# W-Ted/F3D-Gaus

Measured on AMD Instinct MI355X. Metric: rendered views/sec at 256x256 (N Gaussians, K cams), higher is better.
Workload: dtype f32; 1 GPU; C2: 1 image/GPU, 196608 Gaussians (sigma0=0.01), 120-view orbit @256x256, GOF forward raster only; timed region = render + 8-bit RGB frames copied to pinned host memory; compositing arithmetic: fast = error-free float32 pairs for the float64 island + hardware exp/rcp/rsq; every channel within 1e-4 of the oracle (RGB <= 3e-7), EXCEPT that the distortion channel (values 1e-7..1e-5 from cancelling fl; gaussians=196608, views=120, resolution=256, tile_cull=1, views_per_call=120, render_mode=fast, channels=all, parallelism=single GPU

## Files before the change

### f3d-gaus_amd/csrc/f3dg_binning.hip

```cpp
#include "f3dg_common.h"

namespace {

typedef unsigned long long u64;
typedef unsigned int u32;

__global__ void __launch_bounds__(F3DG_BLOCK)
scan_reduce_kernel(const u32* __restrict__ in, u64 n, u32* __restrict__ block_sums)
{
    __shared__ u32 wsum[F3DG_BLOCK / 64];
    const u64 base = (u64)blockIdx.x * F3DG_SCAN_CHUNK;
    u32 s = 0;
#pragma unroll
    for (int i = 0; i < F3DG_SCAN_ITEMS; i++) {
        const u64 k = base + (u64)i * F3DG_BLOCK + threadIdx.x;
        if (k < n) s += in[k];
    }
#pragma unroll
    for (int off = 32; off > 0; off >>= 1) s += __shfl_down(s, off, 64);
    if ((threadIdx.x & 63) == 0) wsum[threadIdx.x >> 6] = s;
    __syncthreads();
    if (threadIdx.x == 0) block_sums[blockIdx.x] = wsum[0] + wsum[1] + wsum[2] + wsum[3];
}

__global__ void __launch_bounds__(1024)
scan_blocksums_kernel(u32* __restrict__ block_sums, u32 nblocks, F3dgHeader* __restrict__ hdr)
{
    __shared__ u32 wtot[16];
    __shared__ u32 carry_s;
    __shared__ u64 carry64_s, wtot64[16];
    if (threadIdx.x == 0) { carry_s = 0; carry64_s = 0; }
    __syncthreads();
    const int lane = threadIdx.x & 63, wave = threadIdx.x >> 6;
    for (u32 start = 0; start < nblocks; start += 1024) {
        const u32 i = start + threadIdx.x;
        const u32 v = i < nblocks ? block_sums[i] : 0;
        u32 x = v;
#pragma unroll
        for (int off = 1; off < 64; off <<= 1) {
            const u32 y = __shfl_up(x, off, 64);
            if (lane >= off) x += y;
        }
        if (lane == 63) wtot[wave] = x;
        unsigned long long v64 = v;
#pragma unroll
        for (int off = 32; off > 0; off >>= 1) v64 += __shfl_down(v64, off, 64);
        if (lane == 0) wtot64[wave] = v64;
        __syncthreads();
        u32 wave_off = 0;
        for (int w = 0; w < wave; w++) wave_off += wtot[w];
        const u32 carry = carry_s;
        if (i < nblocks) block_sums[i] = carry + wave_off + x - v;
        __syncthreads();
        if (threadIdx.x == 1023) {
            carry_s = carry + wave_off + x;
            u64 t = 0;
            for (int w = 0; w < 16; w++) t += wtot64[w];
            carry64_s += t;
        }
        __syncthreads();
    }
    if (hdr && threadIdx.x == 0) {
        const u64 total = carry64_s;
        hdr->num_rendered = total > 0xFFFFFFFFull ? 0xFFFFFFFFu : (u32)total;
        hdr->overflow = total > (u64)hdr->capacity ? 1u : 0u;
    }
}

__global__ void __launch_bounds__(F3DG_BLOCK)
scan_apply_kernel(const u32* in, u32* out , u64 n, const u32* __restrict__ block_sums,
                  int exclusive)
{
    __shared__ u32 wtot[F3DG_BLOCK / 64];
    const u64 base = (u64)blockIdx.x * F3DG_SCAN_CHUNK + (u64)threadIdx.x * F3DG_SCAN_ITEMS;
    u32 v[F3DG_SCAN_ITEMS];
    u32 s = 0;
    if (base + F3DG_SCAN_ITEMS <= n) {
#pragma unroll
        for (int i = 0; i < F3DG_SCAN_ITEMS / 4; i++) {
            const uint4 w = reinterpret_cast<const uint4*>(in + base)[i];
            v[4 * i] = w.x; v[4 * i + 1] = w.y; v[4 * i + 2] = w.z; v[4 * i + 3] = w.w;
        }
    } else {
#pragma unroll
        for (int i = 0; i < F3DG_SCAN_ITEMS; i++) v[i] = (base + i < n) ? in[base + i] : 0;
    }
#pragma unroll
    for (int i = 0; i < F3DG_SCAN_ITEMS; i++) s += v[i];
    const int lane = threadIdx.x & 63, wave = threadIdx.x >> 6;
    u32 x = s;
#pragma unroll
    for (int off = 1; off < 64; off <<= 1) {
        const u32 y = __shfl_up(x, off, 64);
        if (lane >= off) x += y;
    }
    if (lane == 63) wtot[wave] = x;
    __syncthreads();
    u32 run = block_sums[blockIdx.x] + x - s;
    for (int w = 0; w < wave; w++) run += wtot[w];
    u32 o[F3DG_SCAN_ITEMS];
#pragma unroll
    for (int i = 0; i < F3DG_SCAN_ITEMS; i++) {
        const u32 before = run;
        run += v[i];
        o[i] = exclusive ? before : run;
    }
    if (base + F3DG_SCAN_ITEMS <= n) {
#pragma unroll
        for (int i = 0; i < F3DG_SCAN_ITEMS / 4; i++)
            reinterpret_cast<uint4*>(out + base)[i] = make_uint4(o[4 * i], o[4 * i + 1], o[4 * i + 2], o[4 * i + 3]);
    } else {
#pragma unroll
        for (int i = 0; i < F3DG_SCAN_ITEMS; i++)
            if (base + i < n) out[base + i] = o[i];
    }
}


struct SegChunk {
    u64 seg_base;
    u64 obase;
    u32 n;
    u32 cps;
    u32 c;
    u32 seg;
};

struct SegTable {
    const u32* vstart;
    const u32* bglob;
    const u32* xprefix;
    u32 xstride;
    u32 V;
};

struct ShiftDigit {
    int shift;
    u32 mask = 255u;
    __device__ __forceinline__ u32 operator()(u32 k) const { return (k >> shift) & mask; }
};
struct CompactDigit {
    u32 kbase;
    __device__ __forceinline__ u32 operator()(u32 k) const { const u32 d = (k - kbase) >> 16; return d < 255u ? d : 255u; }
};

template <typename K, typename DIGIT, bool MINMAX = false>
__device__ __forceinline__ void hist_chunk(const K* __restrict__ keys, const SegChunk& ck, const DIGIT digit, u32* __restrict__ hist,
                                           u32 (*h)[256], u32* __restrict__ minmax = nullptr)
{
    u32 kmin = 0xFFFFFFFFu, kmax = 0u;
#pragma unroll
    for (int w = 0; w < F3DG_BLOCK / 64; w++) h[w][threadIdx.x] = 0;
    __syncthreads();
    u32* hw = h[threadIdx.x >> 6];
    constexpr int VEC = 16 / (int)sizeof(K);
    typedef K __attribute__((ext_vector_type(VEC))) KV;
    const u64 base = (u64)ck.c * F3DG_SORT_CHUNK;
    const u64 g0 = ck.seg_base + base;
    const u64 g1 = ck.seg_base + ((u64)ck.n - base < (u64)F3DG_SORT_CHUNK ? (u64)ck.n : base + F3DG_SORT_CHUNK);
    for (u64 a = (g0 & ~(u64)(VEC - 1)) + (u64)threadIdx.x * VEC; a < g1; a += (u64)F3DG_BLOCK * VEC) {
        const KV w = *reinterpret_cast<const KV*>(keys + a);
#pragma unroll
        for (int q = 0; q < VEC; q++) {
            if (a + q >= g0 && a + q < g1) {
                const u32 key = (u32)w[q];
                atomicAdd(&hw[digit(key)], 1u);
                if (MINMAX && key != 0xFFFFFFFFu) { kmin = key < kmin ? key : kmin; kmax = key > kmax ? key : kmax; }
            }
        }
    }
    __shared__ u32 wmm[2][F3DG_BLOCK / 64];
    if (MINMAX) {
#pragma unroll
        for (int off = 32; off > 0; off >>= 1) {
            const u32 a = __shfl_down(kmin, off, 64), b = __shfl_down(kmax, off, 64);
            kmin = a < kmin ? a : kmin; kmax = b > kmax ? b : kmax;
        }
        if ((threadIdx.x & 63) == 0) { wmm[0][threadIdx.x >> 6] = kmin; wmm[1][threadIdx.x >> 6] = kmax; }
    }
    __syncthreads();
    if (MINMAX && threadIdx.x == 0) {
        u32 a = wmm[0][0], b = wmm[1][0];
#pragma unroll
        for (int w = 1; w < F3DG_BLOCK / 64; w++) { a = wmm[0][w] < a ? wmm[0][w] : a; b = wmm[1][w] > b ? wmm[1][w] : b; }
        minmax[0] = a; minmax[1] = b;
    }
    hist[ck.obase + (u64)threadIdx.x * ck.cps + ck.c] = h[0][threadIdx.x] + h[1][threadIdx.x] + h[2][threadIdx.x] + h[3][threadIdx.x];
}

struct ScatterShared {
    u32 cnt[F3DG_BLOCK / 64][256];
    u32 lbase[256];
    u32 gdelta[256];
    u32 wtot[F3DG_BLOCK / 64];
    u32 sval[F3DG_SORT_CHUNK];
};

template <typename K, bool IOTA, typename DIGIT>
__device__ __forceinline__ void scatter_chunk(const K* __restrict__ keys_in, const u32* __restrict__ vals_in, K* __restrict__ keys_out,
                                              u32* __restrict__ vals_out, const SegChunk& ck, const DIGIT digit,
                                              const u32* __restrict__ offsets , ScatterShared& sh, K* skey)
{
    const u32 n = ck.n;
    const u64 block_base = (u64)ck.c * F3DG_SORT_CHUNK;
    const u32 in_block = (u32)((n - block_base) < (u64)F3DG_SORT_CHUNK ? (n - block_base) : (u64)F3DG_SORT_CHUNK);
    const int lane = threadIdx.x & 63, wave = threadIdx.x >> 6;
#pragma unroll
    for (int w = 0; w < F3DG_BLOCK / 64; w++) sh.cnt[w][threadIdx.x] = 0;
    __syncthreads();

    const u64 wave_base = block_base + (u64)wave * (64 * F3DG_SORT_ITEMS);
    u32 key[F3DG_SORT_ITEMS];
    u32 val[F3DG_SORT_ITEMS];
    u32 rank[F3DG_SORT_ITEMS];
    const u64 lane_lt = ((u64)1 << lane) - 1;
#pragma unroll
    for (int r = 0; r < F3DG_SORT_ITEMS; r++) {
        const u64 i = wave_base + (u64)r * 64 + lane;
        const bool valid = i < n;
        key[r] = valid ? (u32)keys_in[ck.seg_base + i] : 0u;
        val[r] = IOTA ? (u32)i : (valid ? vals_in[ck.seg_base + i] : 0u);
    }
#pragma unroll
    for (int r = 0; r < F3DG_SORT_ITEMS; r++) {
        const u64 i = wave_base + (u64)r * 64 + lane;
        const bool valid = i < n;
        const u32 d = digit(key[r]);
        u64 diff = 0;
#pragma unroll
        for (int b = 0; b < 8; b++) {
            const u32 own = (u32)((int)(d << (31 - b)) >> 31);
            const u64 bal = __ballot(own != 0u);
            diff |= bal ^ (((u64)own << 32) | own);
        }
        const u64 same = __ballot(valid) & ~diff;
        const u32 below = (u32)__popcll(same & lane_lt);
        const u32 prev = sh.cnt[wave][d];
        rank[r] = prev + below;
        __builtin_amdgcn_wave_barrier();
        if (valid && below == 0) sh.cnt[wave][d] = prev + (u32)__popcll(same);
        __builtin_amdgcn_wave_barrier();
    }
    __syncthreads();
    {
        const u32 d = threadIdx.x;
        const u32 c0 = sh.cnt[0][d], c1 = sh.cnt[1][d], c2 = sh.cnt[2][d], c3 = sh.cnt[3][d];
        const u32 tot = c0 + c1 + c2 + c3;
        u32 x = tot;
#pragma unroll
        for (int off = 1; off < 64; off <<= 1) {
            const u32 y = __shfl_up(x, off, 64);
            if (lane >= off) x += y;
        }
        if (lane == 63) sh.wtot[wave] = x;
        __syncthreads();
        u32 excl = x - tot;
        for (int w = 0; w < wave; w++) excl += sh.wtot[w];
        sh.lbase[d] = excl;
        sh.gdelta[d] = offsets[ck.obase + (u64)d * ck.cps + ck.c] - excl;
        sh.cnt[0][d] = excl;
        sh.cnt[1][d] = excl + c0;
        sh.cnt[2][d] = excl + c0 + c1;
        sh.cnt[3][d] = excl + c0 + c1 + c2;
    }
    __syncthreads();
#pragma unroll
    for (int r = 0; r < F3DG_SORT_ITEMS; r++) {
        const u64 i = wave_base + (u64)r * 64 + lane;
        if (i < n) {
            const u32 d = digit(key[r]);
            const u32 slot = sh.cnt[wave][d] + rank[r];
            skey[slot] = (K)key[r];
            sh.sval[slot] = val[r];
        }
    }
    __syncthreads();
    for (u32 slot = threadIdx.x; slot < in_block; slot += F3DG_BLOCK) {
        const K k = skey[slot];
        const u32 d = digit((u32)k);
        const u32 pos = sh.gdelta[d] + slot;
        if (keys_out) keys_out[pos] = k;
        vals_out[pos] = sh.sval[slot];
    }
}

__device__ __forceinline__ SegChunk fixed_chunk(u32 seg_len, u32 cps)
{
    u32 seg, c;
    f3dg_xcd_map(blockIdx.x, gridDim.x / cps, cps, seg, c);
    SegChunk ck;
    ck.seg_base = (u64)seg * seg_len; ck.obase = (u64)seg * 256u * cps; ck.n = seg_len; ck.cps = cps; ck.c = c; ck.seg = seg;
    return ck;
}

__device__ __forceinline__ bool gsort_compact(const u32* __restrict__ minmax, u32 view, u32& kbase)
{
    const u32 kmin = minmax[2 * view], kmax = minmax[2 * view + 1];
    kbase = kmin & 0xFFFF0000u;
    return kmin <= kmax && ((kmax - kbase) >> 24) == 0u;
}

template <int PASS>
__global__ void __launch_bounds__(F3DG_BLOCK)
gsort_hist_kernel(const u32* __restrict__ keys, u32 seg_len, u32 cps, u32* __restrict__ hist, const u32* __restrict__ minmax,
                  u32* __restrict__ chunk_minmax)
{
    __shared__ u32 h[F3DG_BLOCK / 64][256];
    const SegChunk ck = fixed_chunk(seg_len, cps);
    if constexpr (PASS == 0) {
        hist_chunk<u32, ShiftDigit>(keys, ck, ShiftDigit{0}, hist, h);
    } else if constexpr (PASS == 1) {
        hist_chunk<u32, ShiftDigit, true>(keys, ck, ShiftDigit{8}, hist, h, chunk_minmax + 2 * ((size_t)ck.seg * cps + ck.c));
    } else {
        u32 kbase;
        const bool compact = gsort_compact(minmax, ck.seg, kbase);
        if (!compact) {
            hist_chunk<u32, ShiftDigit>(keys, ck, ShiftDigit{8 * PASS}, hist, h);
        } else if constexpr (PASS == 2) {
            hist_chunk<u32, CompactDigit>(keys, ck, CompactDigit{kbase}, hist, h);
        } else {
            const u64 base = (u64)ck.c * F3DG_SORT_CHUNK;
            const u32 in_chunk = (u32)((ck.n - base) < (u64)F3DG_SORT_CHUNK ? (ck.n - base) : (u64)F3DG_SORT_CHUNK);
            hist[ck.obase + (u64)threadIdx.x * ck.cps + ck.c] = threadIdx.x == 0 ? in_chunk : 0u;
        }
    }
}

__global__ void __launch_bounds__(1024)
gsort_scan_kernel(u32 n_per_seg , u32 seg_len, u32* __restrict__ hist)
{
    __shared__ u32 wtot[16];
    __shared__ u32 carry_s;
    u32* h = hist + (size_t)blockIdx.x * n_per_seg;
    const u32 lane = threadIdx.x & 63u, wave = threadIdx.x >> 6;
    if (threadIdx.x == 0) carry_s = blockIdx.x * seg_len;
    __syncthreads();
    for (u32 base = 0; base < n_per_seg; base += 4096u) {
        const u32 i = base + 4u * threadIdx.x;
        uint4 v = make_uint4(0u, 0u, 0u, 0u);
        if (i < n_per_seg) v = *reinterpret_cast<const uint4*>(h + i);
        const u32 tot = v.x + v.y + v.z + v.w;
        u32 x = tot;
#pragma unroll
        for (int off = 1; off < 64; off <<= 1) {
            const u32 y = __shfl_up(x, off, 64);
            if (lane >= (u32)off) x += y;
        }
        if (lane == 63u) wtot[wave] = x;
        __syncthreads();
        u32 before = carry_s + x - tot;
        for (u32 w = 0; w < wave; w++) before += wtot[w];
        if (i < n_per_seg)
            *reinterpret_cast<uint4*>(h + i) = make_uint4(before, before + v.x, before + v.x + v.y, before + v.x + v.y + v.z);
        __syncthreads();
        if (threadIdx.x == 1023u) carry_s = before + tot;
        __syncthreads();
    }
}

__global__ void __launch_bounds__(64)
gsort_range_kernel(u32 cps, const u32* __restrict__ chunk_minmax, u32* __restrict__ minmax)
{
    u32 kmin = 0xFFFFFFFFu, kmax = 0u;
    for (u32 c = threadIdx.x; c < cps; c += 64) {
        const u32 a = chunk_minmax[2 * ((size_t)blockIdx.x * cps + c)], b = chunk_minmax[2 * ((size_t)blockIdx.x * cps + c) + 1];
        kmin = a < kmin ? a : kmin; kmax = b > kmax ? b : kmax;
    }
#pragma unroll
    for (int off = 32; off > 0; off >>= 1) {
        const u32 a = __shfl_down(kmin, off, 64), b = __shfl_down(kmax, off, 64);
        kmin = a < kmin ? a : kmin; kmax = b > kmax ? b : kmax;
    }
    if (threadIdx.x == 0) { minmax[2 * blockIdx.x] = kmin; minmax[2 * blockIdx.x + 1] = kmax; }
}

template <int PASS>
__global__ void __launch_bounds__(F3DG_BLOCK)
gsort_scatter_kernel(const u32* __restrict__ keys_in, const u32* __restrict__ vals_in, u32* __restrict__ keys_out,
                     u32* __restrict__ vals_out, u32 seg_len, u32 cps, const u32* __restrict__ offsets, const u32* __restrict__ minmax)
{
    __shared__ ScatterShared sh;
    __shared__ u32 skey[F3DG_SORT_CHUNK];
    const SegChunk ck = fixed_chunk(seg_len, cps);
    if constexpr (PASS == 0) {
        scatter_chunk<u32, true, ShiftDigit>(keys_in, vals_in, keys_out, vals_out, ck, ShiftDigit{0}, offsets, sh, skey);
    } else if constexpr (PASS == 1) {
        scatter_chunk<u32, false, ShiftDigit>(keys_in, vals_in, keys_out, vals_out, ck, ShiftDigit{8}, offsets, sh, skey);
    } else {
        u32 kbase;
        const bool compact = gsort_compact(minmax, ck.seg, kbase);
        if (!compact)
            scatter_chunk<u32, false, ShiftDigit>(keys_in, vals_in, PASS == 3 ? (u32*)nullptr : keys_out, vals_out, ck, ShiftDigit{8 * PASS}, offsets, sh, skey);
        else if constexpr (PASS == 2)
            scatter_chunk<u32, false, CompactDigit>(keys_in, vals_in, (u32*)nullptr, vals_out, ck, CompactDigit{kbase}, offsets, sh, skey);
    }
}

__global__ void __launch_bounds__(512)
view_segments_kernel(int V, int P, const u32* __restrict__ offsets_sorted, const F3dgHeader* __restrict__ hdr, u32* __restrict__ vstart,
                     u32* __restrict__ bglob, u32* __restrict__ xprefix, u32 xstride)
{
    __shared__ u32 carry;
    __shared__ u32 wtot[8];
    const u32 lane = threadIdx.x & 63u, wave = threadIdx.x >> 6;
    const bool dead = hdr->overflow != 0;
    auto start_of = [&](u32 v) -> u32 {
        const u64 i = (u64)v * (u64)P;
        return (dead || i == 0) ? 0u : offsets_sorted[i - 1];
    };
    auto chunks_of = [&](u32 v) -> u32 {
        const u32 n = start_of(v + 1) - start_of(v);
        return (n + F3DG_SORT_CHUNK - 1) / F3DG_SORT_CHUNK;
    };
    if (threadIdx.x == 0) carry = 0;
    __syncthreads();
    for (u32 v0 = 0; v0 < (u32)V; v0 += 512) {
        const u32 v = v0 + threadIdx.x;
        const u32 c = v < (u32)V ? chunks_of(v) : 0u;
        u32 x = c;
#pragma unroll
        for (int off = 1; off < 64; off <<= 1) {
            const u32 y = __shfl_up(x, off, 64);
            if (lane >= (u32)off) x += y;
        }
        if (lane == 63) wtot[wave] = x;
        __syncthreads();
        u32 woff = carry;
        for (u32 w = 0; w < wave; w++) woff += wtot[w];
        if (v < (u32)V) { vstart[v] = start_of(v); bglob[v] = woff + x - c; }
        __syncthreads();
        if (threadIdx.x == 511) carry = woff + x;
        __syncthreads();
    }
    if (threadIdx.x == 0) { vstart[V] = start_of((u32)V); bglob[V] = carry; }
    const u32 nk = ((u32)V > wave) ? ((u32)V - wave + 7u) / 8u : 0u;
    u32 run = 0;
    for (u32 k0 = 0; k0 < nk; k0 += 64) {
        const u32 k = k0 + lane;
        const u32 c = k < nk ? chunks_of(wave + 8u * k) : 0u;
        u32 x = c;
#pragma unroll
        for (int off = 1; off < 64; off <<= 1) {
            const u32 y = __shfl_up(x, off, 64);
            if (lane >= (u32)off) x += y;
        }
        if (k < nk) xprefix[wave * xstride + k] = run + x - c;
        run += __shfl(x, 63, 64);
    }
    if (lane == 0) xprefix[wave * xstride + nk] = run;
}

__global__ void __launch_bounds__(F3DG_BLOCK)
ranges_from_offsets_kernel(u32 V, u32 T, int tile_bits, const u32* __restrict__ bglob, const u32* __restrict__ offsets,
                           const F3dgHeader* __restrict__ hdr, uint2* __restrict__ ranges)
{
    const u32 i = blockIdx.x * F3DG_BLOCK + threadIdx.x;
    if (i >= V * T) return;
    const u32 v = i / T, t = i % T;
    const u32 b0 = bglob[v], cpv = bglob[v + 1] - b0;
    uint2 r = make_uint2(0u, 0u);
    if (cpv != 0u && !hdr->overflow) {
        const u32 d = ((v << tile_bits) | t) & 255u;
        const u32 lo = offsets[256ull * b0 + (u64)d * cpv], hi = offsets[256ull * b0 + (u64)(d + 1u) * cpv];
        if (hi > lo) r = make_uint2(lo, hi);
    }
    ranges[i] = r;
}

__device__ __forceinline__ bool var_chunk(const SegTable& st, u32 f, u32& k, SegChunk& ck)
{
    const u32 x = blockIdx.x & 7u;
    const u32* xp = st.xprefix + x * st.xstride;
    const u32 nk = (st.V > x) ? (st.V - x + 7u) / 8u : 0u;
    while (k < nk && f >= xp[k + 1]) k++;
    if (k >= nk) return false;
    const u32 v = x + 8u * k;
    const u32 s0 = st.vstart[v], b0 = st.bglob[v];
    ck.seg_base = s0; ck.n = st.vstart[v + 1] - s0; ck.cps = st.bglob[v + 1] - b0; ck.obase = 256ull * b0; ck.c = f - xp[k];
    return true;
}

template <typename K>
__global__ void __launch_bounds__(F3DG_BLOCK)
radix2_hist_var_kernel(const K* __restrict__ keys, SegTable st, int shift, u32 mask, u32* __restrict__ hist)
{
    __shared__ u32 h[F3DG_BLOCK / 64][256];
    u32 k = 0;
    SegChunk ck;
    for (u32 f = blockIdx.x >> 3; var_chunk(st, f, k, ck); f += gridDim.x >> 3)
        hist_chunk<K, ShiftDigit>(keys, ck, ShiftDigit{shift, mask}, hist, h);
}

template <typename K>
__global__ void __launch_bounds__(F3DG_BLOCK)
radix2_scatter_var_kernel(const K* __restrict__ keys_in, const u32* __restrict__ vals_in, K* __restrict__ keys_out,
                          u32* __restrict__ vals_out, SegTable st, int shift, u32 mask, const u32* __restrict__ offsets)
{
    __shared__ ScatterShared sh;
    __shared__ K skey[F3DG_SORT_CHUNK];
    u32 k = 0;
    SegChunk ck;
    for (u32 f = blockIdx.x >> 3; var_chunk(st, f, k, ck); f += gridDim.x >> 3) {
        scatter_chunk<K, false, ShiftDigit>(keys_in, vals_in, keys_out, vals_out, ck, ShiftDigit{shift, mask}, offsets, sh, skey);
        __syncthreads();
    }
}

__global__ void __launch_bounds__(F3DG_BLOCK)
gsort_gather_rects_kernel(int P, u32* __restrict__ gv0, u32* __restrict__ gv1, const u32* __restrict__ minmax,
                          const uint2* __restrict__ rects, u32* __restrict__ tiles_sorted, u32* __restrict__ rx)
{
    constexpr int ITEMS = 4;
    unsigned view, chunk;
    const unsigned cpv = (unsigned)((P + F3DG_BLOCK * ITEMS - 1) / (F3DG_BLOCK * ITEMS));
    f3dg_xcd_map(blockIdx.x, gridDim.x / cpv, cpv, view, chunk);
    const size_t vb = (size_t)view * P;
    u32 kbase;
    const bool pass2 = gsort_compact(minmax, view, kbase);
    const u32* perm = pass2 ? gv1 : gv0;
    u32* ry = pass2 ? gv0 : gv1;
    const int k0 = (int)(chunk * F3DG_BLOCK * ITEMS + threadIdx.x);
    u32 id[ITEMS];
    uint2 r[ITEMS];
#pragma unroll
    for (int i = 0; i < ITEMS; i++) { const int k = k0 + i * F3DG_BLOCK; id[i] = k < P ? perm[vb + k] : 0u; }
#pragma unroll
    for (int i = 0; i < ITEMS; i++) { const int k = k0 + i * F3DG_BLOCK; r[i] = k < P ? rects[vb + id[i]] : make_uint2(0u, 0u); }
#pragma unroll
    for (int i = 0; i < ITEMS; i++) {
        const int k = k0 + i * F3DG_BLOCK;
        if (k < P) {
            tiles_sorted[vb + k] = (((r[i].x >> 16) & F3DG_RECT_COORD) - (r[i].x & F3DG_RECT_COORD)) *
                                   (((r[i].y >> 16) & F3DG_RECT_COORD) - (r[i].y & F3DG_RECT_COORD));
            rx[vb + k] = r[i].x;
            ry[vb + k] = r[i].y;
        }
    }
}

#define F3DG_DUP_CAP 3072
template <typename G>
__global__ void __launch_bounds__(F3DG_BLOCK)
duplicate_sorted_kernel(int P, int tile_bits, int grid_x, const u32* __restrict__ gv0, const u32* __restrict__ gv1,
                        const u32* __restrict__ minmax, const u32* __restrict__ rx,
                        const u32* __restrict__ offsets_sorted,
                        const F3dgHeader* __restrict__ hdr, G* __restrict__ kgrp, u32* __restrict__ vals)
{
    __shared__ G sk[F3DG_DUP_CAP];
    __shared__ u32 sv[F3DG_DUP_CAP];
    if (hdr->overflow) return;
    const int k = blockIdx.x * F3DG_BLOCK + threadIdx.x;
    const int v = blockIdx.y;
    u32 kbase;
    const bool pass2 = gsort_compact(minmax, (u32)v, kbase);
    const u32* perm = pass2 ? gv1 : gv0;
    const u32* ry = pass2 ? gv0 : gv1;
    const size_t first = (size_t)v * P + (size_t)blockIdx.x * F3DG_BLOCK;
    const int in_block = min(F3DG_BLOCK, P - (int)(blockIdx.x * F3DG_BLOCK));
    const u32 base = first == 0 ? 0u : offsets_sorted[first - 1];
    const u32 n = offsets_sorted[first + in_block - 1] - base;
    u32 off0 = 0, cnt = 0, x = 0, y = 0, g = 0;
    if (k < P) {
        const size_t pos = (size_t)v * P + k;
        x = rx[pos]; y = ry[pos];
        const u32 rminx = x & F3DG_RECT_COORD, rmaxx = (x >> 16) & F3DG_RECT_COORD, rminy = y & F3DG_RECT_COORD, rmaxy = (y >> 16) & F3DG_RECT_COORD;
        if (rmaxx > rminx && rmaxy > rminy) {
            g = perm[pos];
            off0 = ((pos == 0) ? 0 : offsets_sorted[pos - 1]) - base;
            cnt = (rmaxx - rminx) * (rmaxy - rminy);
        }
    }
    const u32 rminx = x & F3DG_RECT_COORD, rmaxx = (x >> 16) & F3DG_RECT_COORD, rminy = y & F3DG_RECT_COORD, rmaxy = (y >> 16) & F3DG_RECT_COORD;
    const u32 view_base = (u32)v << tile_bits;
    auto halves = [](u32 t, u32 tmin, u32 tmax, u32 word) -> u32 {
        u32 m = 3u;
        if (t == tmin && (word & F3DG_RECT_SKIP_LO)) m &= ~1u;
        if (t + 1u == tmax && (word & F3DG_RECT_SKIP_HI)) m &= ~2u;
        return m;
    };
    for (u32 wb = 0; wb < n; wb += (u32)F3DG_DUP_CAP) {
        const u32 lo = off0 > wb ? off0 : wb;
        const u32 hi = off0 + cnt < wb + (u32)F3DG_DUP_CAP ? off0 + cnt : wb + (u32)F3DG_DUP_CAP;
        if (lo < hi) {
            const u32 w = rmaxx - rminx, j0 = lo - off0;
            u32 ty = rminy + j0 / w, tx = rminx + j0 % w;
            u32 my = halves(ty, rminy, rmaxy, y);
            for (u32 j = lo; j < hi; j++) {
                const u32 mx = halves(tx, rminx, rmaxx, x);
                sk[j - wb] = (G)(view_base | (ty * (u32)grid_x + tx));
                sv[j - wb] = g | ((((my & 1u) ? mx : 0u) | ((my & 2u) ? mx << 2 : 0u)) << F3DG_ID_BITS);
                if (++tx == rmaxx) { tx = rminx; ty++; my = halves(ty, rminy, rmaxy, y); }
            }
        }
        __syncthreads();
        const u32 in_win = n - wb < (u32)F3DG_DUP_CAP ? n - wb : (u32)F3DG_DUP_CAP;
        for (u32 i = threadIdx.x; i < in_win; i += F3DG_BLOCK) {
            kgrp[base + wb + i] = sk[i];
            vals[base + wb + i] = sv[i];
        }
        __syncthreads();
    }
}

__global__ void __launch_bounds__(F3DG_BLOCK)
export_keys_kernel(u32 nseg, int P, int tile_bits, int T, const uint2* __restrict__ ranges, const F3dgHeader* __restrict__ hdr,
                   const u32* __restrict__ point_list, const float* __restrict__ depths, u64* __restrict__ keys_out)
{
    if (hdr->overflow) return;
    for (u32 seg = blockIdx.x; seg < nseg; seg += gridDim.x) {
        const uint2 r = ranges[seg];
        const u32 view = seg / (u32)T, tile = seg % (u32)T;
        const u64 hi = (u64)((view << tile_bits) | tile) << 32;
        for (u32 i = r.x + threadIdx.x; i < r.y; i += F3DG_BLOCK)
            keys_out[i] = hi | (u64)__float_as_uint(depths[(size_t)view * P + (point_list[i] & F3DG_ID_MASK)]);
    }
}

template <typename G>
__global__ void __launch_bounds__(F3DG_BLOCK)
group_bounds_kernel(const G* __restrict__ kgrp, const F3dgHeader* __restrict__ hdr, int tile_bits, int T, u32* __restrict__ ranges)
{
    const u32 L = hdr->overflow ? 0u : hdr->num_rendered;
    const u32 tmask = (1u << tile_bits) - 1u;
    for (u64 base = ((u64)blockIdx.x * F3DG_BLOCK + threadIdx.x) * 8u; base < L; base += (u64)gridDim.x * F3DG_BLOCK * 8u) {
        G v[8];
        if (base + 8 <= L) {
            typedef G __attribute__((ext_vector_type(8))) G8;
            const G8 w = *reinterpret_cast<const G8*>(kgrp + base);
#pragma unroll
            for (int i = 0; i < 8; i++) v[i] = w[i];
        } else {
#pragma unroll
            for (int i = 0; i < 8; i++) v[i] = base + i < L ? kgrp[base + i] : (G)0;
        }
        u32 prev = base > 0 ? (u32)kgrp[base - 1] : 0u;
        const u32 next = base + 8 < L ? (u32)kgrp[base + 8] : 0u;
#pragma unroll
        for (int i = 0; i < 8; i++) {
            const u64 idx = base + i;
            if (idx < L) {
                const u32 cur = (u32)v[i];
                const u32 nxt = i < 7 ? (u32)v[i + 1] : next;
                const u32 seg = (cur >> tile_bits) * (u32)T + (cur & tmask);
                if (idx == 0 || prev != cur) ranges[2u * seg] = (u32)idx;
                if (idx == L - 1 || nxt != cur) ranges[2u * seg + 1u] = (u32)idx + 1u;
                prev = cur;
            }
        }
    }
}

int bits_for(unsigned long long n_values)
{
    int b = 0;
    while (b < 64 && (n_values - 1) >> b) b++;
    return n_values <= 1 ? 0 : b;
}

}

int f3dg_launch_scan_inclusive(hipStream_t s, const unsigned* in, unsigned* out, unsigned long long n,
                               unsigned* tmp, unsigned tmp_elems, int exclusive, F3dgHeader* hdr_total)
{
    if (n == 0) return F3DG_OK;
    const unsigned nblocks = (unsigned)((n + F3DG_SCAN_CHUNK - 1) / F3DG_SCAN_CHUNK);
    if (nblocks > tmp_elems) return F3DG_ERR_WORKSPACE;
    F3DG_KLAUNCH(scan_reduce_kernel, dim3(nblocks), dim3(F3DG_BLOCK), 0, s, in, (u64)n, tmp);
    F3DG_KLAUNCH(scan_blocksums_kernel, dim3(1), dim3(1024), 0, s, tmp, nblocks, hdr_total);
    F3DG_KLAUNCH(scan_apply_kernel, dim3(nblocks), dim3(F3DG_BLOCK), 0, s, in, out, (u64)n, tmp, exclusive);
    F3DG_HIP_CHECK(hipGetLastError());
    return F3DG_OK;
}

int f3dg_tile_bits(int T) { return bits_for((unsigned long long)T); }


int f3dg_sort_passes(int V, int T)
{
    (void)V;
    const int bits = f3dg_tile_bits(T);
    return bits == 0 ? 0 : (bits + 7) / 8;
}

template <typename G>
static int binning_tail(hipStream_t s, int V, int P, int grid_x, int T, int tile_bits, const F3dgLayout& L, char* ws, F3dgHeader* hdr)
{
    int rc = F3DG_OK;
    const size_t VP = (size_t)V * P;
    u32* scan_tmp = reinterpret_cast<u32*>(ws + L.scan_tmp);
    u32* hist = reinterpret_cast<u32*>(ws + L.hist);
    u32* gk[2] = { reinterpret_cast<u32*>(ws + L.gsort), reinterpret_cast<u32*>(ws + L.gsort) + VP };
    u32* gv[2] = { reinterpret_cast<u32*>(ws + L.gsort) + 2 * VP, reinterpret_cast<u32*>(ws + L.gsort) + 3 * VP };
    G* kgrp[2] = { reinterpret_cast<G*>(ws + L.keys[0]), reinterpret_cast<G*>(ws + L.keys[1]) };
    u32* vals[2] = { reinterpret_cast<u32*>(ws + L.vals[0]), reinterpret_cast<u32*>(ws + L.vals[1]) };
    const dim3 pgrid((P + F3DG_BLOCK - 1) / F3DG_BLOCK, V);

    const u32 cps = (u32)((P + F3DG_SORT_CHUNK - 1) / F3DG_SORT_CHUNK);
    const u32 gblocks = (u32)V * cps;
    u32* minmax = reinterpret_cast<u32*>(ws + L.segtab) + L.segtab_minmax;
    u32* chunk_minmax = minmax + 2 * (size_t)V;
    const bool view_scan = cps <= 64;
#define F3DG_GSORT_PASS(PASS, IN, OUT)                                                                                                     \
    F3DG_KLAUNCH((gsort_hist_kernel<PASS>), dim3(gblocks), dim3(F3DG_BLOCK), 0, s, gk[IN], (u32)P, cps, hist, minmax, chunk_minmax); \
    if (view_scan)                                                                                                                         \
        F3DG_KLAUNCH(gsort_scan_kernel, dim3(V), dim3(1024), 0, s, 256u * cps, (u32)P, hist);                                       \
    else {                                                                                                                                 \
        rc = f3dg_launch_scan_inclusive(s, hist, hist, (unsigned long long)256 * gblocks, scan_tmp, L.scan_tmp_elems, 1, nullptr);        \
        if (rc != F3DG_OK) return rc;                                                                                                      \
    }                                                                                                                                      \
    F3DG_KLAUNCH((gsort_scatter_kernel<PASS>), dim3(gblocks), dim3(F3DG_BLOCK), 0, s, gk[IN], gv[IN], gk[OUT], gv[OUT], (u32)P, cps, hist, minmax)
    F3DG_GSORT_PASS(0, 0, 1);
    F3DG_GSORT_PASS(1, 1, 0);
    F3DG_KLAUNCH(gsort_range_kernel, dim3(V), dim3(64), 0, s, cps, chunk_minmax, minmax);
    F3DG_GSORT_PASS(2, 0, 1);
    F3DG_GSORT_PASS(3, 1, 0);
#undef F3DG_GSORT_PASS
    u32* offsets_sorted = gk[1];
    u32* rx = gk[0];

    F3DG_KLAUNCH(gsort_gather_rects_kernel, dim3((unsigned)V * (unsigned)((P + 4 * F3DG_BLOCK - 1) / (4 * F3DG_BLOCK))), dim3(F3DG_BLOCK), 0, s, P, gv[0], gv[1], minmax,
                           reinterpret_cast<const uint2*>(ws + L.rects), offsets_sorted, rx);
    rc = f3dg_launch_scan_inclusive(s, offsets_sorted, offsets_sorted, (unsigned long long)VP, scan_tmp, L.scan_tmp_elems, 0, hdr);
    if (rc != F3DG_OK) return rc;
    const int passes = f3dg_sort_passes(V, T);
    int src = passes & 1;
    F3DG_KLAUNCH((duplicate_sorted_kernel<G>), pgrid, dim3(F3DG_BLOCK), 0, s, P, tile_bits, grid_x, gv[0], gv[1], minmax, rx, offsets_sorted, hdr,
                       kgrp[src], vals[src]);

    if (passes > 0) {
        SegTable st;
        u32* segtab = reinterpret_cast<u32*>(ws + L.segtab);
        const u32 xstride = (u32)V / 8u + 2u;
        st.vstart = segtab; st.bglob = segtab + (V + 1); st.xprefix = segtab + 2 * (V + 1); st.xstride = xstride; st.V = (u32)V;
        F3DG_KLAUNCH(view_segments_kernel, dim3(1), dim3(512), 0, s, V, P, offsets_sorted, hdr, segtab, segtab + (V + 1),
                           segtab + 2 * (V + 1), xstride);
        const size_t nbmax = (size_t)L.sort_blocks + (size_t)V;
        const u32 per_xcd = (u32)((nbmax + 7) / 8 < 160 ? (nbmax + 7) / 8 : 160);
        const u32 per_xcd_h = (u32)((nbmax + 7) / 8 < 512 ? (nbmax + 7) / 8 : 512);
        const int split = passes == 2 ? (tile_bits + 1) / 2 : 8;
        for (int p = 0; p < passes; p++) {
            const int shift = split * p;
            const u32 mask = passes == 2 ? (1u << (p == 0 ? split : tile_bits - split)) - 1u : 255u;
            F3DG_HIP_CHECK(hipMemsetAsync(hist, 0, sizeof(u32) * 256 * nbmax, s));
            F3DG_KLAUNCH((radix2_hist_var_kernel<G>), dim3(8 * per_xcd_h), dim3(F3DG_BLOCK), 0, s, kgrp[src], st, shift, mask, hist);
            rc = f3dg_launch_scan_inclusive(s, hist, hist, (unsigned long long)256 * nbmax, scan_tmp, L.scan_tmp_elems, 1, nullptr);
            if (rc != F3DG_OK) return rc;
            F3DG_KLAUNCH((radix2_scatter_var_kernel<G>), dim3(8 * per_xcd), dim3(F3DG_BLOCK), 0, s, kgrp[src], vals[src],
                               passes == 1 ? (G*)nullptr : kgrp[src ^ 1], vals[src ^ 1], st, shift, mask, hist);
            src ^= 1;
        }
        if (passes == 1) {
            const u32 nseg = (u32)V * (u32)T;
            F3DG_KLAUNCH(ranges_from_offsets_kernel, dim3((nseg + F3DG_BLOCK - 1) / F3DG_BLOCK), dim3(F3DG_BLOCK), 0, s, (u32)V, (u32)T, tile_bits,
                               segtab + (V + 1), hist, hdr, reinterpret_cast<uint2*>(ws + L.ranges));
            F3DG_HIP_CHECK(hipGetLastError());
            return F3DG_OK;
        }
    }
    F3DG_HIP_CHECK(hipMemsetAsync(ws + L.ranges, 0, sizeof(uint2) * (size_t)V * T, s));
    F3DG_KLAUNCH((group_bounds_kernel<G>), dim3(2048), dim3(F3DG_BLOCK), 0, s, kgrp[0], hdr, tile_bits, T, reinterpret_cast<u32*>(ws + L.ranges));
    F3DG_HIP_CHECK(hipGetLastError());
    return F3DG_OK;
}

int f3dg_launch_binning(hipStream_t s, int V, int P, int W, int H, const F3dgLayout& L, char* ws, int export_offsets)
{
    const int grid_x = (W + F3DG_TILE - 1) / F3DG_TILE, grid_y = (H + F3DG_TILE - 1) / F3DG_TILE;
    const int T = grid_x * grid_y;
    const int tile_bits = f3dg_tile_bits(T);
    F3dgHeader* hdr = reinterpret_cast<F3dgHeader*>(ws + L.header);

    int rc = F3DG_OK;
    if (export_offsets) {
        rc = f3dg_launch_scan_inclusive(s, reinterpret_cast<const u32*>(ws + L.tiles), reinterpret_cast<u32*>(ws + L.offsets),
                                        (unsigned long long)V * P, reinterpret_cast<u32*>(ws + L.scan_tmp), L.scan_tmp_elems, 0, nullptr);
        if (rc != F3DG_OK) return rc;
    }
    const bool small = (((unsigned long long)(V > 0 ? V - 1 : 0) << tile_bits) | ((1ull << tile_bits) - 1ull)) <= 0xFFFFull;
    rc = small ? binning_tail<unsigned short>(s, V, P, grid_x, T, tile_bits, L, ws, hdr)
               : binning_tail<u32>(s, V, P, grid_x, T, tile_bits, L, ws, hdr);
    if (rc != F3DG_OK) return rc;
    F3DG_HIP_CHECK(hipGetLastError());
    return F3DG_OK;
}

int f3dg_launch_export_keys(hipStream_t s, int V, int P, int W, int H, const F3dgLayout& L, char* ws)
{
    const int grid_x = (W + F3DG_TILE - 1) / F3DG_TILE, grid_y = (H + F3DG_TILE - 1) / F3DG_TILE;
    const int T = grid_x * grid_y;
    const u32 nseg = (u32)V * (u32)T;
    const u32 rg = nseg < 65535u * 4u ? nseg : 65535u * 4u;
    F3DG_KLAUNCH(export_keys_kernel, dim3(rg), dim3(F3DG_BLOCK), 0, s, nseg, P, f3dg_tile_bits(T), T,
                       reinterpret_cast<const uint2*>(ws + L.ranges), reinterpret_cast<const F3dgHeader*>(ws + L.header),
                       reinterpret_cast<const u32*>(ws + L.vals[0]), reinterpret_cast<const float*>(ws + L.depths),
                       reinterpret_cast<u64*>(ws + L.keys[0]));
    F3DG_HIP_CHECK(hipGetLastError());
    return F3DG_OK;
}
```

Baseline: 29990 views/s.

## Replace global per-Gaussian offset scan with block sums and per-view segmented scans

Drops the full V*P inclusive scan of per-Gaussian tile counts. The gather kernel now writes per-block sums, a per-view kernel scans those, view totals feed view_segments, and the duplicate kernel rebuilds intra-block offsets with a wave scan. It also swaps the global scan of the tile radix histograms for a per-view tile_scan kernel, which skips the memset, and skips the redundant pass-3 scan for compact views. The aim is fewer launches and less global memory traffic in binning, at the cost of more complex bookkeeping, overflow detection moved into view_segments, and memset elision that relies on the histogram kernel fully writing its range.

```diff
diff --git a/f3d-gaus_amd/csrc/f3dg_binning.hip b/f3d-gaus_amd/csrc/f3dg_binning.hip
--- a/f3d-gaus_amd/csrc/f3dg_binning.hip
+++ b/f3d-gaus_amd/csrc/f3dg_binning.hip
@@ -303,7 +303,7 @@
 template <int PASS>
 __global__ void __launch_bounds__(F3DG_BLOCK)
 gsort_hist_kernel(const u32* __restrict__ keys, u32 seg_len, u32 cps, u32* __restrict__ hist, const u32* __restrict__ minmax,
-                  u32* __restrict__ chunk_minmax)
+                  u32* __restrict__ chunk_minmax, int standin )
 {
     __shared__ u32 h[F3DG_BLOCK / 64][256];
     const SegChunk ck = fixed_chunk(seg_len, cps);
@@ -318,7 +318,7 @@
             hist_chunk<u32, ShiftDigit>(keys, ck, ShiftDigit{8 * PASS}, hist, h);
         } else if constexpr (PASS == 2) {
             hist_chunk<u32, CompactDigit>(keys, ck, CompactDigit{kbase}, hist, h);
-        } else {
+        } else if (standin) {
             const u64 base = (u64)ck.c * F3DG_SORT_CHUNK;
             const u32 in_chunk = (u32)((ck.n - base) < (u64)F3DG_SORT_CHUNK ? (ck.n - base) : (u64)F3DG_SORT_CHUNK);
             hist[ck.obase + (u64)threadIdx.x * ck.cps + ck.c] = threadIdx.x == 0 ? in_chunk : 0u;
@@ -327,10 +327,12 @@
 }
 
 __global__ void __launch_bounds__(1024)
-gsort_scan_kernel(u32 n_per_seg , u32 seg_len, u32* __restrict__ hist)
+gsort_scan_kernel(u32 n_per_seg , u32 seg_len, u32* __restrict__ hist, const u32* __restrict__ skip_compact )
 {
     __shared__ u32 wtot[16];
     __shared__ u32 carry_s;
+    u32 kbase;
+    if (skip_compact && gsort_compact(skip_compact, blockIdx.x, kbase)) return;
     u32* h = hist + (size_t)blockIdx.x * n_per_seg;
     const u32 lane = threadIdx.x & 63u, wave = threadIdx.x >> 6;
     if (threadIdx.x == 0) carry_s = blockIdx.x * seg_len;
@@ -396,20 +398,87 @@
     }
 }
 
+
+__global__ void __launch_bounds__(1024)
+block_sums_scan_kernel(u32 nb, u32* __restrict__ block_sums, u64* __restrict__ view_total)
+{
+    __shared__ u32 wtot[16];
+    __shared__ u32 carry_s;
+    __shared__ u64 carry64_s, wtot64[16];
+    u32* b = block_sums + (size_t)blockIdx.x * nb;
+    const u32 lane = threadIdx.x & 63u, wave = threadIdx.x >> 6;
+    if (threadIdx.x == 0) { carry_s = 0; carry64_s = 0; }
+    __syncthreads();
+    for (u32 start = 0; start < nb; start += 1024u) {
+        const u32 i = start + threadIdx.x;
+        const u32 v = i < nb ? b[i] : 0u;
+        u32 x = v;
+#pragma unroll
+        for (int off = 1; off < 64; off <<= 1) {
+            const u32 y = __shfl_up(x, off, 64);
+            if (lane >= (u32)off) x += y;
+        }
+        if (lane == 63u) wtot[wave] = x;
+        u64 v64 = v;
+#pragma unroll
+        for (int off = 32; off > 0; off >>= 1) v64 += __shfl_down(v64, off, 64);
+        if (lane == 0u) wtot64[wave] = v64;
+        __syncthreads();
+        u32 before = carry_s + x - v;
+        for (u32 w = 0; w < wave; w++) before += wtot[w];
+        if (i < nb) b[i] = before;
+        __syncthreads();
+        if (threadIdx.x == 1023u) {
+            carry_s = before + v;
+            u64 t = 0;
+            for (int w = 0; w < 16; w++) t += wtot64[w];
+            carry64_s += t;
+        }
+        __syncthreads();
+    }
+    if (threadIdx.x == 0) view_total[blockIdx.x] = carry64_s;
+}
+
 __global__ void __launch_bounds__(512)
-view_segments_kernel(int V, int P, const u32* __restrict__ offsets_sorted, const F3dgHeader* __restrict__ hdr, u32* __restrict__ vstart,
+view_segments_kernel(int V, const u64* __restrict__ view_total, F3dgHeader* __restrict__ hdr, u32* __restrict__ vstart,
                      u32* __restrict__ bglob, u32* __restrict__ xprefix, u32 xstride)
 {
     __shared__ u32 carry;
     __shared__ u32 wtot[8];
+    __shared__ u64 carry64, wtot64[8];
     const u32 lane = threadIdx.x & 63u, wave = threadIdx.x >> 6;
-    const bool dead = hdr->overflow != 0;
-    auto start_of = [&](u32 v) -> u32 {
-        const u64 i = (u64)v * (u64)P;
-        return (dead || i == 0) ? 0u : offsets_sorted[i - 1];
-    };
+    if (threadIdx.x == 0) carry64 = 0;
+    __syncthreads();
+    for (u32 v0 = 0; v0 < (u32)V; v0 += 512) {
+        const u32 v = v0 + threadIdx.x;
+        const u64 t = v < (u32)V ? view_total[v] : 0ull;
+        u64 x = t;
+#pragma unroll
+        for (int off = 1; off < 64; off <<= 1) {
+            const u64 y = __shfl_up(x, off, 64);
+            if (lane >= (u32)off) x += y;
+        }
+        if (lane == 63) wtot64[wave] = x;
+        __syncthreads();
+        u64 woff = carry64;
+        for (u32 w = 0; w < wave; w++) woff += wtot64[w];
+        if (v < (u32)V) vstart[v] = (u32)(woff + x - t);
+        __syncthreads();
+        if (threadIdx.x == 511) carry64 = woff + x;
+        __syncthreads();
+    }
+    const u64 total = carry64;
+    const bool dead = total > (u64)hdr->capacity;
+    if (threadIdx.x == 0) {
+        hdr->num_rendered = total > 0xFFFFFFFFull ? 0xFFFFFFFFu : (u32)total;
+        hdr->overflow = dead ? 1u : 0u;
+        vstart[V] = dead ? 0u : (u32)total;
+    }
+    if (dead)
+        for (u32 v = threadIdx.x; v < (u32)V; v += 512) vstart[v] = 0u;
+    __syncthreads();
     auto chunks_of = [&](u32 v) -> u32 {
-        const u32 n = start_of(v + 1) - start_of(v);
+        const u32 n = vstart[v + 1] - vstart[v];
         return (n + F3DG_SORT_CHUNK - 1) / F3DG_SORT_CHUNK;
     };
     if (threadIdx.x == 0) carry = 0;
@@ -427,12 +496,12 @@
         __syncthreads();
         u32 woff = carry;
         for (u32 w = 0; w < wave; w++) woff += wtot[w];
-        if (v < (u32)V) { vstart[v] = start_of(v); bglob[v] = woff + x - c; }
+        if (v < (u32)V) bglob[v] = woff + x - c;
         __syncthreads();
         if (threadIdx.x == 511) carry = woff + x;
         __syncthreads();
     }
-    if (threadIdx.x == 0) { vstart[V] = start_of((u32)V); bglob[V] = carry; }
+    if (threadIdx.x == 0) bglob[V] = carry;
     const u32 nk = ((u32)V > wave) ? ((u32)V - wave + 7u) / 8u : 0u;
     u32 run = 0;
     for (u32 k0 = 0; k0 < nk; k0 += 64) {
@@ -448,6 +517,53 @@
         run += __shfl(x, 63, 64);
     }
     if (lane == 0) xprefix[wave * xstride + nk] = run;
+}
+
+__global__ void __launch_bounds__(1024)
+tile_scan_kernel(u32 V, const u32* __restrict__ vstart, const u32* __restrict__ bglob, u32* __restrict__ hist)
+{
+    constexpr u32 ITEMS = 16;
+    __shared__ u32 wtot[16];
+    __shared__ u32 carry_s;
+    const u32 b0 = bglob[blockIdx.x], n = 256u * (bglob[blockIdx.x + 1] - b0);
+    u32* h = hist + 256ull * b0;
+    const u32 lane = threadIdx.x & 63u, wave = threadIdx.x >> 6;
+    if (blockIdx.x == 0 && threadIdx.x == 0) hist[256ull * bglob[V]] = vstart[V];
+    if (threadIdx.x == 0) carry_s = vstart[blockIdx.x];
+    __syncthreads();
+    for (u32 base = 0; base < n; base += 1024u * ITEMS) {
+        const u32 i = base + ITEMS * threadIdx.x;
+        u32 v[ITEMS];
+#pragma unroll
+        for (u32 q = 0; q < ITEMS / 4; q++) {
+            const uint4 w = i < n ? reinterpret_cast<const uint4*>(h + i)[q] : make_uint4(0u, 0u, 0u, 0u);
+            v[4 * q] = w.x; v[4 * q + 1] = w.y; v[4 * q + 2] = w.z; v[4 * q + 3] = w.w;
+        }
+        u32 tot = 0;
+#pragma unroll
+        for (u32 q = 0; q < ITEMS; q++) tot += v[q];
+        u32 x = tot;
+#pragma unroll
+        for (int off = 1; off < 64; off <<= 1) {
+            const u32 y = __shfl_up(x, off, 64);
+            if (lane >= (u32)off) x += y;
+        }
+        if (lane == 63u) wtot[wave] = x;
+        __syncthreads();
+        u32 run = carry_s + x - tot;
+        for (u32 w = 0; w < wave; w++) run += wtot[w];
+        if (i < n) {
+#pragma unroll
+            for (u32 q = 0; q < ITEMS / 4; q++) {
+                uint4 o;
+                o.x = run; run += v[4 * q]; o.y = run; run += v[4 * q + 1]; o.z = run; run += v[4 * q + 2]; o.w = run; run += v[4 * q + 3];
+                reinterpret_cast<uint4*>(h + i)[q] = o;
+            }
+        }
+        __syncthreads();
+        if (threadIdx.x == 1023u) carry_s = run;
+        __syncthreads();
+    }
 }
 
 __global__ void __launch_bounds__(F3DG_BLOCK)
@@ -506,11 +622,18 @@
     }
 }
 
+__device__ __forceinline__ u32 rect_instances(u32 x, u32 y)
+{
+    const u32 rminx = x & F3DG_RECT_COORD, rmaxx = (x >> 16) & F3DG_RECT_COORD, rminy = y & F3DG_RECT_COORD, rmaxy = (y >> 16) & F3DG_RECT_COORD;
+    return (rmaxx > rminx && rmaxy > rminy) ? (rmaxx - rminx) * (rmaxy - rminy) : 0u;
+}
+
 __global__ void __launch_bounds__(F3DG_BLOCK)
 gsort_gather_rects_kernel(int P, u32* __restrict__ gv0, u32* __restrict__ gv1, const u32* __restrict__ minmax,
-                          const uint2* __restrict__ rects, u32* __restrict__ tiles_sorted, u32* __restrict__ rx)
+                          const uint2* __restrict__ rects, u32* __restrict__ block_sums, u32* __restrict__ rx)
 {
     constexpr int ITEMS = 4;
+    __shared__ u32 wsum[ITEMS][F3DG_BLOCK / 64];
     unsigned view, chunk;
     const unsigned cpv = (unsigned)((P + F3DG_BLOCK * ITEMS - 1) / (F3DG_BLOCK * ITEMS));
     f3dg_xcd_map(blockIdx.x, gridDim.x / cpv, cpv, view, chunk);
@@ -530,12 +653,19 @@
     for (int i = 0; i < ITEMS; i++) {
         const int k = k0 + i * F3DG_BLOCK;
         if (k < P) {
-            tiles_sorted[vb + k] = (((r[i].x >> 16) & F3DG_RECT_COORD) - (r[i].x & F3DG_RECT_COORD)) *
-                                   (((r[i].y >> 16) & F3DG_RECT_COORD) - (r[i].y & F3DG_RECT_COORD));
             rx[vb + k] = r[i].x;
             ry[vb + k] = r[i].y;
         }
-    }
+        u32 sum = rect_instances(r[i].x, r[i].y);
+#pragma unroll
+        for (int off = 32; off > 0; off >>= 1) sum += __shfl_down(sum, off, 64);
+        if ((threadIdx.x & 63) == 0) wsum[i][threadIdx.x >> 6] = sum;
+    }
+    __syncthreads();
+    const unsigned nb = (unsigned)((P + F3DG_BLOCK - 1) / F3DG_BLOCK);
+    const unsigned blk = chunk * ITEMS + threadIdx.x;
+    if (threadIdx.x < ITEMS && blk < nb)
+        block_sums[(size_t)view * nb + blk] = wsum[threadIdx.x][0] + wsum[threadIdx.x][1] + wsum[threadIdx.x][2] + wsum[threadIdx.x][3];
 }
 
 #define F3DG_DUP_CAP 3072
@@ -543,11 +673,12 @@
 __global__ void __launch_bounds__(F3DG_BLOCK)
 duplicate_sorted_kernel(int P, int tile_bits, int grid_x, const u32* __restrict__ gv0, const u32* __restrict__ gv1,
                         const u32* __restrict__ minmax, const u32* __restrict__ rx,
-                        const u32* __restrict__ offsets_sorted,
+                        const u32* __restrict__ block_base , const u32* __restrict__ vstart ,
                         const F3dgHeader* __restrict__ hdr, G* __restrict__ kgrp, u32* __restrict__ vals)
 {
     __shared__ G sk[F3DG_DUP_CAP];
     __shared__ u32 sv[F3DG_DUP_CAP];
+    __shared__ u32 wtot[F3DG_BLOCK / 64];
     if (hdr->overflow) return;
     const int k = blockIdx.x * F3DG_BLOCK + threadIdx.x;
     const int v = blockIdx.y;
@@ -555,20 +686,28 @@
     const bool pass2 = gsort_compact(minmax, (u32)v, kbase);
     const u32* perm = pass2 ? gv1 : gv0;
     const u32* ry = pass2 ? gv0 : gv1;
-    const size_t first = (size_t)v * P + (size_t)blockIdx.x * F3DG_BLOCK;
-    const int in_block = min(F3DG_BLOCK, P - (int)(blockIdx.x * F3DG_BLOCK));
-    const u32 base = first == 0 ? 0u : offsets_sorted[first - 1];
-    const u32 n = offsets_sorted[first + in_block - 1] - base;
-    u32 off0 = 0, cnt = 0, x = 0, y = 0, g = 0;
+    const u32 base = (vstart ? vstart[v] : 0u) + block_base[(size_t)v * gridDim.x + blockIdx.x];
+    u32 cnt = 0, x = 0, y = 0, g = 0;
     if (k < P) {
         const size_t pos = (size_t)v * P + k;
         x = rx[pos]; y = ry[pos];
-        const u32 rminx = x & F3DG_RECT_COORD, rmaxx = (x >> 16) & F3DG_RECT_COORD, rminy = y & F3DG_RECT_COORD, rmaxy = (y >> 16) & F3DG_RECT_COORD;
-        if (rmaxx > rminx && rmaxy > rminy) {
-            g = perm[pos];
-            off0 = ((pos == 0) ? 0 : offsets_sorted[pos - 1]) - base;
-            cnt = (rmaxx - rminx) * (rmaxy - rminy);
-        }
+        cnt = rect_instances(x, y);
+        if (cnt) g = perm[pos];
+    }
+    u32 off0, n;
+    {
+        const int lane = threadIdx.x & 63, wave = threadIdx.x >> 6;
+        u32 incl = cnt;
+#pragma unroll
+        for (int off = 1; off < 64; off <<= 1) {
+            const u32 t = __shfl_up(incl, off, 64);
+            if (lane >= off) incl += t;
+        }
+        if (lane == 63) wtot[wave] = incl;
+        __syncthreads();
+        off0 = incl - cnt;
+        for (int w = 0; w < wave; w++) off0 += wtot[w];
+        n = wtot[0] + wtot[1] + wtot[2] + wtot[3];
     }
     const u32 rminx = x & F3DG_RECT_COORD, rmaxx = (x >> 16) & F3DG_RECT_COORD, rminy = y & F3DG_RECT_COORD, rmaxy = (y >> 16) & F3DG_RECT_COORD;
     const u32 view_base = (u32)v << tile_bits;
@@ -701,9 +840,9 @@
     u32* chunk_minmax = minmax + 2 * (size_t)V;
     const bool view_scan = cps <= 64;
 #define F3DG_GSORT_PASS(PASS, IN, OUT)                                                                                                     \
-    F3DG_KLAUNCH((gsort_hist_kernel<PASS>), dim3(gblocks), dim3(F3DG_BLOCK), 0, s, gk[IN], (u32)P, cps, hist, minmax, chunk_minmax); \
+    F3DG_KLAUNCH((gsort_hist_kernel<PASS>), dim3(gblocks), dim3(F3DG_BLOCK), 0, s, gk[IN], (u32)P, cps, hist, minmax, chunk_minmax, view_scan ? 0 : 1); \
     if (view_scan)                                                                                                                         \
-        F3DG_KLAUNCH(gsort_scan_kernel, dim3(V), dim3(1024), 0, s, 256u * cps, (u32)P, hist);                                       \
+        F3DG_KLAUNCH(gsort_scan_kernel, dim3(V), dim3(1024), 0, s, 256u * cps, (u32)P, hist, PASS == 3 ? minmax : (const u32*)nullptr); \
     else {                                                                                                                                 \
         rc = f3dg_launch_scan_inclusive(s, hist, hist, (unsigned long long)256 * gblocks, scan_tmp, L.scan_tmp_elems, 1, nullptr);        \
         if (rc != F3DG_OK) return rc;                                                                                                      \
@@ -715,36 +854,46 @@
     F3DG_GSORT_PASS(2, 0, 1);
     F3DG_GSORT_PASS(3, 1, 0);
 #undef F3DG_GSORT_PASS
-    u32* offsets_sorted = gk[1];
+    u32* block_sums = gk[1];
     u32* rx = gk[0];
+    u64* view_total = reinterpret_cast<u64*>(chunk_minmax);
+    const u32 nb = (u32)((P + F3DG_BLOCK - 1) / F3DG_BLOCK);
+    SegTable st;
+    u32* segtab = reinterpret_cast<u32*>(ws + L.segtab);
+    const u32 xstride = (u32)V / 8u + 2u;
+    st.vstart = segtab; st.bglob = segtab + (V + 1); st.xprefix = segtab + 2 * (V + 1); st.xstride = xstride; st.V = (u32)V;
 
     F3DG_KLAUNCH(gsort_gather_rects_kernel, dim3((unsigned)V * (unsigned)((P + 4 * F3DG_BLOCK - 1) / (4 * F3DG_BLOCK))), dim3(F3DG_BLOCK), 0, s, P, gv[0], gv[1], minmax,
-                           reinterpret_cast<const uint2*>(ws + L.rects), offsets_sorted, rx);
-    rc = f3dg_launch_scan_inclusive(s, offsets_sorted, offsets_sorted, (unsigned long long)VP, scan_tmp, L.scan_tmp_elems, 0, hdr);
-    if (rc != F3DG_OK) return rc;
+                           reinterpret_cast<const uint2*>(ws + L.rects), block_sums, rx);
     const int passes = f3dg_sort_passes(V, T);
+    if (passes > 0) {
+        F3DG_KLAUNCH(block_sums_scan_kernel, dim3(V), dim3(1024), 0, s, nb, block_sums, view_total);
+        F3DG_KLAUNCH(view_segments_kernel, dim3(1), dim3(512), 0, s, V, view_total, hdr, segtab, segtab + (V + 1), segtab + 2 * (V + 1), xstride);
+    } else {
+        rc = f3dg_launch_scan_inclusive(s, block_sums, block_sums, (unsigned long long)V * nb, scan_tmp, L.scan_tmp_elems, 1, hdr);
+        if (rc != F3DG_OK) return rc;
+    }
     int src = passes & 1;
-    F3DG_KLAUNCH((duplicate_sorted_kernel<G>), pgrid, dim3(F3DG_BLOCK), 0, s, P, tile_bits, grid_x, gv[0], gv[1], minmax, rx, offsets_sorted, hdr,
-                       kgrp[src], vals[src]);
+    F3DG_KLAUNCH((duplicate_sorted_kernel<G>), pgrid, dim3(F3DG_BLOCK), 0, s, P, tile_bits, grid_x, gv[0], gv[1], minmax, rx, block_sums,
+                       passes > 0 ? segtab : (const u32*)nullptr, hdr, kgrp[src], vals[src]);
 
     if (passes > 0) {
-        SegTable st;
-        u32* segtab = reinterpret_cast<u32*>(ws + L.segtab);
-        const u32 xstride = (u32)V / 8u + 2u;
-        st.vstart = segtab; st.bglob = segtab + (V + 1); st.xprefix = segtab + 2 * (V + 1); st.xstride = xstride; st.V = (u32)V;
-        F3DG_KLAUNCH(view_segments_kernel, dim3(1), dim3(512), 0, s, V, P, offsets_sorted, hdr, segtab, segtab + (V + 1),
-                           segtab + 2 * (V + 1), xstride);
         const size_t nbmax = (size_t)L.sort_blocks + (size_t)V;
         const u32 per_xcd = (u32)((nbmax + 7) / 8 < 160 ? (nbmax + 7) / 8 : 160);
         const u32 per_xcd_h = (u32)((nbmax + 7) / 8 < 512 ? (nbmax + 7) / 8 : 512);
+        const bool tile_view_scan = nbmax <= (size_t)512 * (size_t)V;
         const int split = passes == 2 ? (tile_bits + 1) / 2 : 8;
         for (int p = 0; p < passes; p++) {
             const int shift = split * p;
             const u32 mask = passes == 2 ? (1u << (p == 0 ? split : tile_bits - split)) - 1u : 255u;
-            F3DG_HIP_CHECK(hipMemsetAsync(hist, 0, sizeof(u32) * 256 * nbmax, s));
+            if (!tile_view_scan) F3DG_HIP_CHECK(hipMemsetAsync(hist, 0, sizeof(u32) * 256 * nbmax, s));
             F3DG_KLAUNCH((radix2_hist_var_kernel<G>), dim3(8 * per_xcd_h), dim3(F3DG_BLOCK), 0, s, kgrp[src], st, shift, mask, hist);
-            rc = f3dg_launch_scan_inclusive(s, hist, hist, (unsigned long long)256 * nbmax, scan_tmp, L.scan_tmp_elems, 1, nullptr);
-            if (rc != F3DG_OK) return rc;
+            if (tile_view_scan)
+                F3DG_KLAUNCH(tile_scan_kernel, dim3(V), dim3(1024), 0, s, (u32)V, st.vstart, st.bglob, hist);
+            else {
+                rc = f3dg_launch_scan_inclusive(s, hist, hist, (unsigned long long)256 * nbmax, scan_tmp, L.scan_tmp_elems, 1, nullptr);
+                if (rc != F3DG_OK) return rc;
+            }
             F3DG_KLAUNCH((radix2_scatter_var_kernel<G>), dim3(8 * per_xcd), dim3(F3DG_BLOCK), 0, s, kgrp[src], vals[src],
                                passes == 1 ? (G*)nullptr : kgrp[src ^ 1], vals[src ^ 1], st, shift, mask, hist);
             src ^= 1;
```

New measurement: 31340 views/s, median of 6. +4.5%, better.
